# adamyindh/Multi-Step-Actor-Critic-Learning-with-Lyapunov-Certificates-for-Exponentially-Stabilizing-Control

Measured on NVIDIA B200. Metric: fused rollout env-steps/sec, higher is better.
Workload: dtype bf16x3 (split-bf16 tensor-core products, f32 accumulate; f32/f64 dynamics)

## Files before the change

include/msacl_b200.h:

```cpp
#ifndef MSACL_B200_H_
#define MSACL_B200_H_

#include <stdint.h>

#ifdef __cplusplus
extern "C" {
#endif

#define MSACL_ABI_VERSION 2

enum {
  MSACL_ENV_VANDERPOL = 0,
  MSACL_ENV_PENDULUM = 1,
  MSACL_ENV_DUCTEDFAN = 2,
  MSACL_ENV_TWOLINK = 3,
  MSACL_ENV_SINGLETRACKCAR = 4,
  MSACL_ENV_QUADTRACKING = 5,
  MSACL_NUM_ENVS = 6
};

enum {
  MSACL_OK = 0,
  MSACL_ERR_BAD_ENV = -1,
  MSACL_ERR_BAD_ARG = -2,
// ... 156 lines not shown
                             const float* dxq1, const float* dxq2, const float* log_alpha, const float* old_act,
                             const float* old_logp, const float* adv, float clip_coef, const float* act_low, const float* act_high,
                             float min_log_std, float max_log_std, float* grad_logits, double* sums, void* stream);
int msacl_alpha_update(float* log_alpha, const double* sums, int64_t rows, float target_entropy, float* adam_state,
                       float one_minus_beta1, float beta2, float one_minus_beta2, float step_size, float bc2_sqrt, float eps,
                       float clamp_max, float* entropy_out, const float* dyn, void* stream);
int msacl_adam_multi(int32_t count, float* const* params, const float* const* grads, float* const* exp_avg, float* const* exp_avg_sq,
                     const int64_t* numel, const int32_t* nsplit, int64_t max_numel, float one_minus_beta1, float beta2,
                     float one_minus_beta2, float step_size, float bc2_sqrt, float eps, const float* dyn, void* stream);
int msacl_adam_tick(int32_t* step, float* dyn, double lr, double beta1, double beta2, void* stream);

int msacl_ffma_probe(int32_t mode, int32_t iters, float* sink, double* flops, void* stream);

int msacl_selftest_tc_gemm(const float* A, const float* W, float* D, int32_t splits, void* stream);

int msacl_umma_probe(int32_t mode, int32_t iters, double* cycles_per_umma, void* stream);

enum {
  MSACL_CERT_NONFINITE = 1,
  MSACL_CERT_BOUND_LO = 2,
  MSACL_CERT_BOUND_HI = 4,
  MSACL_CERT_DECREASE = 8,
  MSACL_CERT_ESCAPED = 16,
  MSACL_CERT_NOT_EXP_STABLE = 32,
  MSACL_CERT_FAIL_MASK = 31,
  MSACL_CERT_MAX_HORIZON = 8192
};

enum {
  MSACL_CERT_SUM_STATES = 0,
// ... 119 lines not shown
```

multi-step-actor-critic-learning-with-lyapunov-certificates-for-exponentially-stabilizing-control_b200/_lib.py:

```python
import ctypes as C
import os

from . import build as _build

_LIB = None
ABI_VERSION = 2

c_f32p = C.POINTER(C.c_float)
c_f64p = C.POINTER(C.c_double)
c_i32p = C.POINTER(C.c_int32)
c_i64p = C.POINTER(C.c_int64)
c_u8p = C.POINTER(C.c_uint8)
vp = C.c_void_p


class EnvState(C.Structure):
    _fields_ = [("env_id", C.c_int32), ("max_step", C.c_int32), ("n", C.c_int64), ("stride", C.c_int64),
                ("sf", vp), ("sd", vp), ("step", vp), ("episode", vp), ("ep_return", vp), ("ep_len", vp),
                ("run", vp), ("seed", C.c_uint64), ("env_base", C.c_uint64)]


class Actor(C.Structure):
    _fields_ = [("w1", vp), ("b1", vp), ("w2t", vp), ("b2", vp), ("w3", vp), ("b3", vp),
                ("min_log_std", C.c_float), ("max_log_std", C.c_float)]
# ... 81 lines not shown
    "msacl_selftest_quad_polar": (C.c_int, [vp, vp, C.c_int64, C.c_float, vp]),
    "msacl_window_store": (C.c_int, [C.POINTER(Transitions), C.c_int32, C.c_int32, C.c_int64, C.POINTER(Ring), vp, vp,
                                     vp, vp]),
    "msacl_window_index_store": (C.c_int, [vp, C.c_int32, C.c_int64, C.c_int64, vp, C.c_int64, vp, vp, vp, vp]),
    "msacl_window_gather_indexed": (C.c_int, [C.POINTER(Transitions), C.c_int64, vp, vp, C.c_int64, C.POINTER(Ring), vp]),
    "msacl_ring_sample": (C.c_int, [C.POINTER(Ring), vp, C.c_uint64, C.c_uint64, C.c_int64, C.POINTER(Ring), vp, vp]),
    "msacl_window_sample_indexed": (C.c_int, [C.POINTER(Transitions), C.c_int64, vp, C.c_int64, vp, vp, C.c_int32, C.c_uint64, C.c_uint64,
                                              C.c_int64, C.POINTER(Ring), vp, vp]),
    "msacl_ring_gather": (C.c_int, [C.POINTER(Ring), vp, C.c_int64, C.POINTER(Ring), vp]),
    "msacl_q_backup": (C.c_int, [C.c_int64, vp, vp, vp, vp, vp, C.c_float, C.c_float, vp, vp]),
    "msacl_lyapunov_risk": (C.c_int, [C.c_int64, C.c_int32, C.c_int32, vp, vp, vp, vp, vp, vp, vp, vp, vp, C.c_float,
                                      C.c_float, C.c_float, C.c_float, vp, vp, vp, vp, vp, vp]),
    "msacl_stability_advantage": (C.c_int, [C.c_int64, C.c_int32, vp, vp, vp, vp, vp, vp, vp]),
    "msacl_advantage_normalize": (C.c_int, [C.c_int64, vp, vp, vp, vp]),
    "msacl_selftest_tc_gemm": (C.c_int, [vp, vp, vp, C.c_int32, vp]),
    "msacl_polyak_update": (C.c_int, [C.c_int32, vp, vp, vp, C.c_int64, C.c_float, C.c_float, vp]),
    "msacl_gemm_tc": (C.c_int, [C.POINTER(Gemm), vp]),
    "msacl_gemm_packed_b_bytes": (C.c_int64, [i32, i32]),
    "msacl_gemm_pack_b": (C.c_int, [C.POINTER(Gemm), vp, vp]),
    "msacl_colsum": (C.c_int, [vp, i64, i32, i64, i32, vp, vp]),
    "msacl_concat2": (C.c_int, [vp, i32, vp, i32, i64, vp, vp]),
    "msacl_reduce_splits": (C.c_int, [vp, i64, i32, vp, vp]),
    "msacl_tanh_gauss_rsample": (C.c_int, [i64, i32, vp, vp, vp, vp, f32, f32, vp, vp, vp]),
    "msacl_tanh_gauss_log_prob": (C.c_int, [i64, i32, vp, vp, vp, vp, f32, f32, vp, vp]),
    "msacl_tanh_gauss_log_prob_bwd": (C.c_int, [i64, i32, vp, vp, vp, vp, f32, f32, vp, i32, vp, vp]),
    "msacl_q_backup_dev_alpha": (C.c_int, [i64, vp, vp, vp, vp, vp, f32, vp, vp, vp]),
    "msacl_q_loss_grad": (C.c_int, [i64, vp, vp, vp, vp, vp, vp, vp]),
    "msacl_sumsq_bwd": (C.c_int, [i64, i32, vp, vp, vp, vp]),
    "msacl_policy_q_route": (C.c_int, [i64, vp, vp, vp, vp, vp, vp, vp, vp]),
    "msacl_policy_logits_grad": (C.c_int, [i64, i32, i32, i32, vp, vp, vp, vp, vp, vp, vp, vp, f32, vp, vp, f32, f32, vp, vp, vp]),
# ... 67 lines not shown
```

multi-step-actor-critic-learning-with-lyapunov-certificates-for-exponentially-stabilizing-control_b200/csrc/rollout_tc.cu:

```cuda
#include "env_phase.cuh"
#include "tcgen05.cuh"

namespace msacl {

#ifdef MSACL_TC_TIMING
#define TC_T0(var) const long long var = clock64()
#define TC_ACC(slot, t0) do { if (stats) atomicAdd(&stats[slot], (double)(clock64() - (t0))); } while (0)
#else
#define TC_T0(var) do {} while (0)
#define TC_ACC(slot, t0) do {} while (0)
#endif

#ifdef MSACL_TC_WATCHDOG
__device__ __forceinline__ void wd_wait(void* bar, uint32_t parity, int site, uint32_t aux, double* stats) {
  const long long t0 = clock64();
  uint32_t spins = 0;
  volatile unsigned long long* flag = reinterpret_cast<volatile unsigned long long*>(&stats[24]);
  while (!tc::mbar_test(bar, parity)) {
    if ((++spins & 1023u) == 0u) {
      if (*flag != 0ull) return;
      if (clock64() - t0 > 3000000000LL) {
        if (atomicCAS(reinterpret_cast<unsigned long long*>(&stats[24]), 0ull, 0x3FF0000000000000ull) == 0ull) {
          stats[25] = site; stats[26] = aux; stats[27] = blockIdx.x; stats[28] = parity; stats[29] = threadIdx.x;
          __threadfence();
// ... 15 lines not shown
constexpr int NCH = TC_HID / KC2;
constexpr int KCB = 16;
constexpr int NCHB = TC_HID / KCB;
constexpr int NB_MAX = 4;
constexpr int A_HALF = TCM * KC2 * 2;
constexpr int B_HALF = TC_HID * KCB * 2;
constexpr int A_LBO = TCM * 16, B_LBO = TC_HID * 16, SBO = 128;
constexpr int X_HALF = TCM * 16 * 2;
constexpr int W1_HALF = TC_HID * 16 * 2;
constexpr int TC_THREADS = 768, TC_ENV_REGS = 112, TC_EPI_REGS = 56, TC_MISC_REGS = 32;
constexpr int W2P_BYTES = NCHB * 2 * B_HALF;
constexpr int W1P_BYTES = 2 * W1_HALF;

struct TcBars {
  unsigned long long xfull[TC_NS], logits[TC_NS];
  unsigned long long h1full[2], h1free[2], h2full[2], h2free[2];
  unsigned long long afull[NCH], afree[NCH], bfull[NB_MAX], bfree[NB_MAX];
  uint32_t tmem_slot;
};

struct TcShare {
  int64_t first;
  int share, rounds, per, ex;
  __host__ __device__ TcShare(int64_t num_tiles, int64_t G, int64_t cta, int nt_max) {
    share = (int)(num_tiles / G + (cta < num_tiles % G ? 1 : 0));
    first = cta * (num_tiles / G) + (cta < num_tiles % G ? cta : num_tiles % G);
    rounds = (share + nt_max - 1) / nt_max;
    per = rounds ? share / rounds : 0;
    ex = rounds ? share % rounds : 0;
  }
  __host__ __device__ int tiles_in_round(int j) const { return per + (j < ex ? 1 : 0); }
// ... 3 lines not shown
template <int ID> __host__ __device__ constexpr bool tc_two_kblocks() { return Env<ID>::D + 1 > 8; }
template <int ID> __host__ __device__ constexpr int tc_ring_depth() { return tc_two_kblocks<ID>() ? 3 : 4; }
template <int ID> __host__ __device__ constexpr int tc_w3_stride() { return 2 * Env<ID>::A > 4 ? 8 : 4; }

template <int ID>
struct TcSmem {
  static constexpr bool X2 = tc_two_kblocks<ID>();
  static constexpr int NB = tc_ring_depth<ID>();
  static constexpr int XH = X2 ? X_HALF : X_HALF / 2;
  static constexpr int W1H = X2 ? W1_HALF : W1_HALF / 2;
  alignas(128) unsigned char bstage[NB][2 * B_HALF];
  alignas(128) unsigned char astage[NCH][2 * A_HALF];
  alignas(128) unsigned char w1p[2 * W1H];
  alignas(128) unsigned char xop[TC_NS][2 * XH];
  alignas(128) unsigned char zeros[X2 ? 128 : W1_HALF / 2];
  alignas(16) float w3t[TC_HID * tc_w3_stride<ID>()];
  alignas(16) float b2[TC_HID];
  alignas(16) float b3[8];
  TcBars bars;
};

typedef unsigned long long u64;
__device__ __forceinline__ u64 pack2(float lo, float hi) { u64 r; asm("mov.b64 %0, {%1, %2};" : "=l"(r) : "f"(lo), "f"(hi)); return r; }
__device__ __forceinline__ void unpack2(u64 v, float& lo, float& hi) { asm("mov.b64 {%0, %1}, %2;" : "=f"(lo), "=f"(hi) : "l"(v)); }
__device__ __forceinline__ u64 fma2(u64 a, u64 b, u64 c) { u64 d; asm("fma.rn.f32x2 %0, %1, %2, %3;" : "=l"(d) : "l"(a), "l"(b), "l"(c)); return d; }

__device__ __forceinline__ uint32_t pack_bf16x2_rn(float lo, float hi) {
  uint32_t r;
  asm("cvt.rn.bf16x2.f32 %0, %1, %2;" : "=r"(r) : "f"(hi), "f"(lo));
  return r;
}
__device__ __forceinline__ void split8(const float (&v)[8], uint4& hi, uint4& lo) {
  uint32_t h[4], l[4];
#pragma unroll
  for (int p = 0; p < 4; ++p) {
    h[p] = pack_bf16x2_rn(v[2 * p], v[2 * p + 1]);
    const float r0 = v[2 * p] - __uint_as_float(h[p] << 16);
    const float r1 = v[2 * p + 1] - __uint_as_float(h[p] & 0xFFFF0000u);
    l[p] = pack_bf16x2_rn(r0, r1);
  }
  hi = make_uint4(h[0], h[1], h[2], h[3]);
  lo = make_uint4(l[0], l[1], l[2], l[3]);
}

__global__ void tc_pack_actor_kernel(msacl_actor_t actor, int D, unsigned char* __restrict__ w1p, unsigned char* __restrict__ w2p) {
  const int gid = blockIdx.x * blockDim.x + threadIdx.x;
  if (gid < NCHB * 2 * TC_HID) {
    const int n = gid % TC_HID, kb = (gid / TC_HID) % 2, c = gid / (TC_HID * 2);
    float v[8];
#pragma unroll
    for (int j = 0; j < 8; ++j) v[j] = actor.w2t[(size_t)(c * KCB + kb * 8 + j) * TC_HID + n];
    uint4 hi, lo;
    split8(v, hi, lo);
    unsigned char* base = w2p + (size_t)c * 2 * B_HALF + kb * B_LBO + n * 16;
// ... 18 lines not shown

template <int ID>
__global__ void __launch_bounds__(TC_THREADS, 1)
rollout_tc_kernel(msacl_env_state_t st, msacl_actor_t actor, const unsigned char* __restrict__ w1p_g,
                  const unsigned char* __restrict__ w2p_g, int K, uint32_t step_base, int n_step,
                  float reward_scale, float cost_scale, const float* __restrict__ eps, int deterministic, msacl_transitions_t out,
                  double* stats) {
  using E = Env<ID>;
  using S = TcSmem<ID>;
  constexpr int D = E::D, A = E::A, A2 = 2 * A;
  constexpr int NS = TC_NS;
  constexpr int NB = S::NB, XH = S::XH, W1H = S::W1H, W3S = tc_w3_stride<ID>();
  constexpr bool X2 = S::X2;
  constexpr int W_EPI1 = 4 * NS, W_MMA = W_EPI1 + 8, W_TMA = W_MMA + 1;
  static_assert(D < 16, "layer-1 K block holds obs + bias column");
  static_assert(A2 * TCM * 4 <= XH && ((A2 + 1) / 2) * 2 * TCM * 4 <= XH, "logits and partial sums alias the two halves of the X-operand region");
  extern __shared__ __align__(128) unsigned char smem_raw[];
  S& sm = *reinterpret_cast<S*>(smem_raw);
  const int tid = threadIdx.x, lane = tid & 31, warp = tid >> 5;
  auto logits_of = [&](int s) { return reinterpret_cast<float*>(sm.xop[s]); };

  for (int i = tid; i < 2 * W1H / 16; i += TC_THREADS) {
    const int img = i / (W1H / 16), off = i % (W1H / 16);
    reinterpret_cast<uint4*>(sm.w1p)[i] = reinterpret_cast<const uint4*>(w1p_g + (size_t)img * W1_HALF)[off];
  }
  for (int i = tid; i < (int)sizeof(sm.zeros) / 16; i += TC_THREADS) reinterpret_cast<uint4*>(sm.zeros)[i] = make_uint4(0, 0, 0, 0);
  for (int i = tid; i < W3S * TC_HID; i += TC_THREADS) { const int n = i / W3S, j = i % W3S; sm.w3t[i] = j < A2 ? actor.w3[j * TC_HID + n] : 0.f; }
  for (int i = tid; i < TC_HID; i += TC_THREADS) sm.b2[i] = actor.b2[i];
  if (tid < 8) sm.b3[tid] = tid < A2 ? actor.b3[tid] : 0.f;
  if (tid == 0) {
    TcBars& b = sm.bars;
    for (int s = 0; s < NS; ++s) tc::mbar_init(&b.xfull[s], TCM);
    for (int s = 0; s < NS; ++s) tc::mbar_init(&b.logits[s], TCM);
    for (int i = 0; i < 2; ++i) {
      tc::mbar_init(&b.h1full[i], 1); tc::mbar_init(&b.h1free[i], 2 * TCM);
      tc::mbar_init(&b.h2full[i], 1); tc::mbar_init(&b.h2free[i], 2 * TCM);
    }
    for (int i = 0; i < NCH; ++i) { tc::mbar_init(&b.afull[i], TCM); tc::mbar_init(&b.afree[i], 1); }
    for (int i = 0; i < NB; ++i) { tc::mbar_init(&b.bfull[i], 1); tc::mbar_init(&b.bfree[i], 1); }
    tc::mbar_fence_init();
  }
  if (warp == W_MMA) tc::tmem_alloc(&sm.bars.tmem_slot, 512);
  tc::fence_async_smem();
  tc::tc_fence_before();
  __syncthreads();
  tc::tc_fence_after();
  const uint32_t tmem = sm.bars.tmem_slot;

  const int64_t num_tiles = (st.n + TCM - 1) / TCM;
  const int64_t G = gridDim.x, cta = blockIdx.x;
  const TcShare sh(num_tiles, G, cta, NS);
// ... 113 lines not shown
          *reinterpret_cast<uint4*>(base + kb * A_LBO) = hi;
          *reinterpret_cast<uint4*>(base + A_HALF + kb * A_LBO) = lo;
        }
        tc::fence_async_smem();
        tc::mbar_arrive(&sm.bars.afull[c]);
      }
      if (timer) TC_ACC(9, t_b);
    };
    auto epi2 = [&](uint32_t t0, int s) {
      const uint32_t buf = t0 & 1u, tmem_b = tmem + buf * 256u;
      TC_T0(t_a);
      TC_WAIT(&sm.bars.h2full[buf], (t0 >> 1) & 1, 4, t0);
      tc::tc_fence_after();
      if (timer) TC_ACC(11, t_a);
      TC_T0(t_b);
      constexpr int NP = (A2 + 1) / 2;
      u64 acc[NP];
#pragma unroll
      for (int p = 0; p < NP; ++p) acc[p] = h == 0 ? pack2(sm.b3[2 * p], sm.b3[2 * p + 1]) : pack2(0.f, 0.f);
#pragma unroll 1
      for (int cc = 0; cc < TC_HID / 32; ++cc) {
        const int cb = h * (TC_HID / 32) + cc;
        uint32_t v[16];
        tc::tmem_ld16(tmem_b + lane_addr + (uint32_t)(cb * 16), v);
        tc::tmem_ld_wait();
        if (cc == TC_HID / 32 - 1) { tc::tc_fence_before(); tc::mbar_arrive(&sm.bars.h2free[buf]); }
#pragma unroll
        for (int g = 0; g < 4; ++g) {
          const float4 bb = *reinterpret_cast<const float4*>(&sm.b2[cb * 16 + 4 * g]);
          const float hv[4] = {fmaxf(__uint_as_float(v[4 * g + 0]) + bb.x, 0.f), fmaxf(__uint_as_float(v[4 * g + 1]) + bb.y, 0.f),
                               fmaxf(__uint_as_float(v[4 * g + 2]) + bb.z, 0.f), fmaxf(__uint_as_float(v[4 * g + 3]) + bb.w, 0.f)};
#pragma unroll
          for (int c = 0; c < 4; ++c) {
            const float* wrow = &sm.w3t[(cb * 16 + 4 * g + c) * W3S];
            const u64 hh = pack2(hv[c], hv[c]);
            if constexpr (NP >= 1) {
              const float4 w0 = *reinterpret_cast<const float4*>(wrow);
              acc[0] = fma2(hh, pack2(w0.x, w0.y), acc[0]);
              if constexpr (NP >= 2) acc[1] = fma2(hh, pack2(w0.z, w0.w), acc[1]);
            }
            if constexpr (NP >= 3) {
              const float4 w1 = *reinterpret_cast<const float4*>(wrow + 4);
              acc[2] = fma2(hh, pack2(w1.x, w1.y), acc[2]);
              if constexpr (NP >= 4) acc[3] = fma2(hh, pack2(w1.z, w1.w), acc[3]);
            }
          }
        }
      }
      float* part = reinterpret_cast<float*>(sm.xop[s] + XH);
      float* lgs = logits_of(s);
      if (h == 1) {
#pragma unroll
        for (int p = 0; p < NP; ++p) {
          float lo, hi;
          unpack2(acc[p], lo, hi);
          part[(2 * p) * TCM + r] = lo;
          part[(2 * p + 1) * TCM + r] = hi;
        }
      }
      tc::bar_sync(4 + q, 64);
      if (h == 0) {
#pragma unroll
        for (int p = 0; p < NP; ++p) {
          float lo, hi;
          unpack2(acc[p], lo, hi);
          lgs[(2 * p) * TCM + r] = lo + part[(2 * p) * TCM + r];
          if (2 * p + 1 < A2) lgs[(2 * p + 1) * TCM + r] = hi + part[(2 * p + 1) * TCM + r];
        }
        tc::mbar_arrive(&sm.bars.logits[s]);
      }
      if (timer) TC_ACC(12, t_b);
    };
    uint32_t ts = 0;
    for (int64_t pair = blockIdx.x; pair < num_pairs; pair += gridDim.x) {
      const int nt = tiles_in_pair(pair);
      for (int k = 0; k < K; ++k)
        for (int s = 0; s < nt; ++s, ++ts) {
          if (ts == 0) epi1(0u);
          const bool has_next = !(s + 1 == nt && k + 1 == K && pair + (int64_t)gridDim.x >= num_pairs);
          const bool epi2_first = nt <= 1;
          if (!epi2_first) {
            if (has_next) epi1(ts + 1);
            epi2(ts, s);
          } else {
            epi2(ts, s);
            if (has_next) epi1(ts + 1);
// ... 18 lines not shown
        TC_T0(t_x);
        TC_WAIT(&sm.bars.xfull[s % NS], xn & 1, 7, t1);
        TC_ACC(13, t_x);
        tc::tc_fence_after();
        const uint32_t tmem_b = tmem + (t1 & 1u) * 256u;
        const uint32_t xbase = tc::smem_u32(sm.xop[s % NS]), zbase = tc::smem_u32(sm.zeros);
        const uint64_t dw1 = tc::make_smem_desc(w1base, X2 ? B_LBO : zbase - w1base, SBO);
        const uint64_t dw2 = tc::make_smem_desc(w1base + W1H, X2 ? B_LBO : zbase - (w1base + W1H), SBO);
        const uint64_t dx1 = tc::make_smem_desc(xbase, X2 ? A_LBO : zbase - xbase, SBO);
        const uint64_t dx2 = tc::make_smem_desc(xbase + XH, X2 ? A_LBO : zbase - (xbase + XH), SBO);
        tc::umma_bf16(tmem_b, dx1, dw1, idesc, 0u);
        tc::umma_bf16(tmem_b, dx1, dw2, idesc, 1u);
        tc::umma_bf16(tmem_b, dx2, dw1, idesc, 1u);
        tc::umma_commit(&sm.bars.h1full[t1 & 1]);
      };
      uint32_t ts = 0, pi = 0;
      for (int64_t pair = blockIdx.x; pair < num_pairs; pair += gridDim.x, ++pi) {
        const int nt = tiles_in_pair(pair);
        for (int k = 0; k < K; ++k)
          for (int s = 0; s < nt; ++s, ++ts) {
            if (ts == 0) issue_l1(0, 0u, 0u);
            const uint32_t buf = ts & 1u, tmem_b = tmem + buf * 256u;
            int s2 = s + 1, k2 = k;
            int64_t pair2 = pair;
            uint32_t pi2 = pi;
            if (s2 == nt) { s2 = 0; if (++k2 == K) { k2 = 0; pair2 += gridDim.x; ++pi2; } }
            bool next_pending = pair2 < num_pairs;
            const uint32_t xn2 = x_index(pi2, k2, s2, (pair2 == pair || !next_pending) ? nt : tiles_in_pair(pair2)), t2 = ts + 1;
            auto try_next = [&]() {
              if (next_pending && (t2 < 2 || tc::mbar_test(&sm.bars.h2free[t2 & 1], ((t2 >> 1) - 1) & 1)) &&
                  tc::mbar_test(&sm.bars.xfull[s2 % NS], xn2 & 1)) {
                issue_l1(s2, xn2, t2);
                next_pending = false;
              }
            };
            try_next();
            TC_T0(t_h);
            TC_WAIT(&sm.bars.h1free[buf], (ts >> 1) & 1, 8, ts);
            TC_ACC(14, t_h);
#pragma unroll 1
            for (int c = 0; c < NCH; ++c) {
              TC_T0(t_1);
              TC_WAIT(&sm.bars.afull[c], ts & 1, 9, ts);
              TC_ACC(15, t_1);
              const uint32_t a_lo = a_lo0 + (uint32_t)c * (2 * A_HALF / 16);
#pragma unroll
              for (int j = 0; j < KC2 / KCB; ++j) {
                TC_T0(t_2);
                TC_WAIT(&sm.bars.bfull[bs], bph, 11, ts);
                TC_ACC(16, t_2);
                tc::tc_fence_after();
                const uint32_t b_lo = b_lo0 + bs * (2 * B_HALF / 16);
                const uint64_t da1 = mk(a_lo + j * (2 * A_LBO / 16)), da2 = mk(a_lo + j * (2 * A_LBO / 16) + A_HALF / 16);
                const uint64_t db1 = mk(b_lo), db2 = mk(b_lo + B_HALF / 16);
                tc::umma_bf16(tmem_b, da1, db1, idesc, (c > 0 || j > 0) ? 1u : 0u);
                tc::umma_bf16(tmem_b, da1, db2, idesc, 1u);
                tc::umma_bf16(tmem_b, da2, db1, idesc, 1u);
                tc::umma_commit(&sm.bars.bfree[bs]);
                if (++bs == NB) { bs = 0; bph ^= 1u; }
              }
              tc::umma_commit(&sm.bars.afree[c]);
              try_next();
            }
            tc::umma_commit(&sm.bars.h2full[buf]);
            if (next_pending) issue_l1(s2, xn2, t2);
#ifdef MSACL_TC_TIMING
            if (stats) atomicAdd(&stats[18], 1.0);
#endif
          }
      }
    }
    } else if (warp == W_TMA) {
    if (tc::elect_one()) {
      int64_t tile_steps = 0;
      for (int64_t pair = blockIdx.x; pair < num_pairs; pair += gridDim.x) tile_steps += (int64_t)tiles_in_pair(pair) * K;
      const int64_t total = tile_steps * NCHB;
      uint32_t bs = 0, bph = 1, kk = 0;
      for (int64_t i = 0; i < total; ++i) {
        if (i >= NB) TC_WAIT(&sm.bars.bfree[bs], bph, 13, i);
// ... 66 lines not shown
```

multi-step-actor-critic-learning-with-lyapunov-certificates-for-exponentially-stabilizing-control_b200/csrc/tc_selftest.cu:

```cuda
#include "common.cuh"
#include "tcgen05.cuh"

namespace msacl {

constexpr int ST_M = 128, ST_N = 256, ST_K = 256, ST_KC = 64;

__global__ void __launch_bounds__(128, 1)
tc_gemm_selftest_kernel(const float* __restrict__ A, const float* __restrict__ W, float* __restrict__ D, int splits) {
  extern __shared__ __align__(128) unsigned char smem[];
  unsigned char* a1 = smem;
  unsigned char* a2 = smem + 65536;
  unsigned char* b1 = smem + 131072;
  unsigned char* b2 = smem + 131072 + 32768;
  unsigned long long* bar = reinterpret_cast<unsigned long long*>(smem + 196608);
  uint32_t* tmem_slot = reinterpret_cast<uint32_t*>(smem + 196608 + 64);
  const int tid = threadIdx.x, warp = tid >> 5, lane = tid & 31;

  if (tid == 0) { tc::mbar_init(bar, 1); tc::mbar_fence_init(); }
  if (warp == 0) tc::tmem_alloc(tmem_slot, 256);
  tc::tc_fence_before();
  __syncthreads();
  tc::tc_fence_after();
  const uint32_t tmem = *tmem_slot;

// ... 39 lines not shown
    tc::mbar_wait(bar, (uint32_t)(c & 1));
    tc::tc_fence_after();
  }
  for (int cb = 0; cb < ST_N / 32; ++cb) {
    uint32_t r[32];
    tc::tmem_ld32(tmem + ((uint32_t)(warp * 32) << 16) + (uint32_t)(cb * 32), r);
    tc::tmem_ld_wait();
#pragma unroll
    for (int j = 0; j < 32; ++j) D[(warp * 32 + lane) * ST_N + cb * 32 + j] = __uint_as_float(r[j]);
  }
  tc::tc_fence_before();
  __syncthreads();
  if (warp == 0) tc::tmem_dealloc(tmem, 256);
}

__global__ void __launch_bounds__(256, 1) umma_probe_kernel(int mode, int iters, double* __restrict__ out) {
  extern __shared__ __align__(128) unsigned char smem[];
  unsigned char* a = smem;
  unsigned char* b = smem + 131072;
  unsigned char* scratch = smem + 180224;
  unsigned long long* bar = reinterpret_cast<unsigned long long*>(smem + 204800);
  uint32_t* tmem_slot = reinterpret_cast<uint32_t*>(smem + 204800 + 64);
  volatile int* stop = reinterpret_cast<volatile int*>(smem + 204800 + 128);
  const int tid = threadIdx.x, warp = tid >> 5;
  unsigned long long* ldcount = reinterpret_cast<unsigned long long*>(smem + 204800 + 192);
  for (int i = tid; i < 180224 / 16; i += 256) reinterpret_cast<uint4*>(smem)[i] = make_uint4(0, 0, 0, 0);
  if (tid == 0) { tc::mbar_init(bar, 1); tc::mbar_init(bar + 1, 1); tc::mbar_init(bar + 2, 1); tc::mbar_fence_init(); tc::mbar_arrive(bar + 2); *stop = 0; *ldcount = 0ull; }
  if (warp == 0) tc::tmem_alloc(tmem_slot, 512);
  tc::fence_async_smem();
  tc::tc_fence_before();
  __syncthreads();
  tc::tc_fence_after();
  const uint32_t tmem = *tmem_slot;
  if (tid == 0) {
    const uint32_t idesc = tc::make_idesc_bf16(128, 256);
    const long long t0 = clock64();
    for (int i = 0; i < iters; ++i) {
      const uint32_t ab = tc::smem_u32(a + ((i >> 1) & 7) * 16384 + (i & 1) * 4096), bb = tc::smem_u32(b + (i % 3) * 16384);
      const uint64_t da1 = tc::make_smem_desc(ab, 2048, 128), da2 = tc::make_smem_desc(ab + 8192, 2048, 128);
      const uint64_t db1 = tc::make_smem_desc(bb, 4096, 128), db2 = tc::make_smem_desc(bb + 8192, 4096, 128);
      tc::umma_bf16(tmem, da1, db1, idesc, i > 0 ? 1u : 0u);
      tc::umma_bf16(tmem, da1, db2, idesc, 1u);
      tc::umma_bf16(tmem, da2, db1, idesc, 1u);
      if (mode >= 3) tc::umma_commit(bar + 1);
      if (mode >= 4) { tc::mbar_wait(bar + 2, 0u); tc::tc_fence_after(); }
    }
    tc::umma_commit(bar);
    tc::mbar_wait(bar, 0u);
    const long long t1 = clock64();
    *stop = 1;
    if (blockIdx.x == 0) { out[0] = (double)(t1 - t0) / (3.0 * iters); out[2] = (double)(t1 - t0); }
  } else if (warp > 0 && warp < 4 && mode == 1) {
    uint4 v = make_uint4(tid, tid, tid, tid);
    int off = (tid - 32) * 16;
    while (!*stop) {
#pragma unroll
      for (int q = 0; q < 8; ++q) *reinterpret_cast<uint4*>(scratch + ((off + q * 1536) % 24576)) = v;
      off = (off + 12288) % 24576;
    }
  } else if (warp > 0 && mode == 2) {
    unsigned long long n = 0;
    uint32_t acc = 0;
    while (!*stop) {
#pragma unroll 1
      for (int cb = 0; cb < 8; ++cb) {
        uint32_t v[32];
// ... 6 lines not shown
    }
    if (acc == 0x12345678u) out[3] = 1.0;
    if ((tid & 31) == 0) atomicAdd(ldcount, n);
  }
  tc::tc_fence_before();
  __syncthreads();
  if (tid == 0 && blockIdx.x == 0 && mode == 2) out[1] = (double)(*ldcount) * 4096.0 / out[2];
  if (warp == 0) tc::tmem_dealloc(tmem, 512);
}

}

using namespace msacl;

extern "C" int msacl_umma_probe(int32_t mode, int32_t iters, double* cycles_per_umma, void* stream) {
  if (!cycles_per_umma || iters <= 0 || mode < 0 || mode > 4) { set_error("umma_probe: bad argument"); return MSACL_ERR_BAD_ARG; }
  const int smem = 204800 + 256;
  cudaError_t e = cudaFuncSetAttribute(umma_probe_kernel, cudaFuncAttributeMaxDynamicSharedMemorySize, smem);
  if (e != cudaSuccess) { set_error("umma_probe: %s", cudaGetErrorString(e)); return MSACL_ERR_CUDA; }
  umma_probe_kernel<<<kNumSMs, 256, smem, (cudaStream_t)stream>>>(mode, iters, cycles_per_umma);
  return check_launch("umma_probe");
}

extern "C" int msacl_selftest_tc_gemm(const float* A, const float* W, float* D, int32_t splits, void* stream) {
  if (!A || !W || !D || (splits != 1 && splits != 3)) { set_error("selftest_tc_gemm: bad argument"); return MSACL_ERR_BAD_ARG; }
  const int smem = 196608 + 128;
  cudaError_t e = cudaFuncSetAttribute(tc_gemm_selftest_kernel, cudaFuncAttributeMaxDynamicSharedMemorySize, smem);
  if (e != cudaSuccess) { set_error("selftest_tc_gemm: %s", cudaGetErrorString(e)); return MSACL_ERR_CUDA; }
  tc_gemm_selftest_kernel<<<1, 128, smem, (cudaStream_t)stream>>>(A, W, D, splits);
  return check_launch("selftest_tc_gemm");
}
```

multi-step-actor-critic-learning-with-lyapunov-certificates-for-exponentially-stabilizing-control_b200/csrc/tcgen05.cuh:

```cuda
#pragma once
#include <cstdint>

namespace msacl {
namespace tc {

__device__ __forceinline__ uint32_t smem_u32(const void* p) { return (uint32_t)__cvta_generic_to_shared(p); }

__device__ __forceinline__ bool elect_one() {
  uint32_t pred;
  asm volatile(
      "{\n\t"
      ".reg .pred p;\n\t"
      "elect.sync _|p, 0xffffffff;\n\t"
      "selp.u32 %0, 1, 0, p;\n\t"
      "}" : "=r"(pred));
  return pred != 0;
}

__device__ __forceinline__ void mbar_init(void* bar, uint32_t count) {
  asm volatile("mbarrier.init.shared::cta.b64 [%0], %1;" ::"r"(smem_u32(bar)), "r"(count) : "memory");
}
__device__ __forceinline__ void mbar_fence_init() {
  asm volatile("fence.mbarrier_init.release.cluster;" ::: "memory");
}
// ... 57 lines not shown
}
__host__ __device__ constexpr uint32_t make_idesc_bf16(int M, int N) {
  return (1u << 4)
         | (1u << 7) | (1u << 10)
         | ((uint32_t)(N >> 3) << 17)
         | ((uint32_t)(M >> 4) << 24);
}

__device__ __forceinline__ void umma_bf16(uint32_t tmem_d, uint64_t a_desc, uint64_t b_desc, uint32_t idesc, uint32_t accumulate) {
  asm volatile(
      "{\n\t"
      ".reg .pred p;\n\t"
      "setp.ne.b32 p, %4, 0;\n\t"
      "tcgen05.mma.cta_group::1.kind::f16 [%0], %1, %2, %3, p;\n\t"
      "}" ::"r"(tmem_d), "l"(a_desc), "l"(b_desc), "r"(idesc), "r"(accumulate) : "memory");
}
__device__ __forceinline__ void umma_commit(void* bar) {
  asm volatile("tcgen05.commit.cta_group::1.mbarrier::arrive::one.shared::cluster.b64 [%0];" ::"r"(smem_u32(bar)) : "memory");
}

__device__ __forceinline__ void tmem_ld32(uint32_t taddr, uint32_t (&r)[32]) {
  asm volatile(
      "tcgen05.ld.sync.aligned.32x32b.x32.b32 "
      "{%0, %1, %2, %3, %4, %5, %6, %7, %8, %9, %10, %11, %12, %13, %14, %15, "
      "%16, %17, %18, %19, %20, %21, %22, %23, %24, %25, %26, %27, %28, %29, %30, %31}, [%32];"
      : "=r"(r[0]), "=r"(r[1]), "=r"(r[2]), "=r"(r[3]), "=r"(r[4]), "=r"(r[5]), "=r"(r[6]), "=r"(r[7]), "=r"(r[8]),
        "=r"(r[9]), "=r"(r[10]), "=r"(r[11]), "=r"(r[12]), "=r"(r[13]), "=r"(r[14]), "=r"(r[15]), "=r"(r[16]),
        "=r"(r[17]), "=r"(r[18]), "=r"(r[19]), "=r"(r[20]), "=r"(r[21]), "=r"(r[22]), "=r"(r[23]), "=r"(r[24]),
        "=r"(r[25]), "=r"(r[26]), "=r"(r[27]), "=r"(r[28]), "=r"(r[29]), "=r"(r[30]), "=r"(r[31])
      : "r"(taddr)
// ... 10 lines not shown
}
__device__ __forceinline__ void tmem_ld8(uint32_t taddr, uint32_t (&r)[8]) {
  asm volatile(
      "tcgen05.ld.sync.aligned.32x32b.x8.b32 {%0, %1, %2, %3, %4, %5, %6, %7}, [%8];"
      : "=r"(r[0]), "=r"(r[1]), "=r"(r[2]), "=r"(r[3]), "=r"(r[4]), "=r"(r[5]), "=r"(r[6]), "=r"(r[7])
      : "r"(taddr)
      : "memory");
}
__device__ __forceinline__ void tmem_ld_wait() { asm volatile("tcgen05.wait::ld.sync.aligned;" ::: "memory"); }
__device__ __forceinline__ void tmem_st8(uint32_t taddr, const uint32_t (&r)[8]) {
  asm volatile(
      "tcgen05.st.sync.aligned.32x32b.x8.b32 [%0], {%1, %2, %3, %4, %5, %6, %7, %8};"
      ::"r"(taddr), "r"(r[0]), "r"(r[1]), "r"(r[2]), "r"(r[3]), "r"(r[4]), "r"(r[5]), "r"(r[6]), "r"(r[7])
      : "memory");
}
__device__ __forceinline__ void tmem_st_wait() { asm volatile("tcgen05.wait::st.sync.aligned;" ::: "memory"); }

__device__ __forceinline__ uint32_t f32_to_bf16_bits(float x) {
  uint32_t u = __float_as_uint(x);
  u += 0x7FFFu + ((u >> 16) & 1u);
  return u >> 16;
}
__device__ __forceinline__ void split_bf16(float x, uint32_t& hi, uint32_t& lo) {
  hi = f32_to_bf16_bits(x);
  const float r = x - __uint_as_float(hi << 16);
  lo = f32_to_bf16_bits(r);
}

}
}
```

Baseline: 2.155 billion.

## Move actor layer-3 matmul onto tensor cores with TMEM A-operand

Replaces the CUDA-core FMA loop for the actor's third layer with tcgen05 MMAs. The epilogue warps apply bias and ReLU to layer-2 outputs, split them into bf16 hi/lo, and store them back into TMEM. The MMA warp then issues M=128,N=16 MMAs with TMEM as the A operand against a packed hi/lo W3 image in shared memory. The first K block is still done on CUDA cores in the slot where the accumulator lands. New l3full/l3done barriers and opportunistic issue points in the MMA loop add synchronisation and extra tensor-core work. This trades epilogue FMA cost for TMEM round trips and serialization risk.

```diff
diff --git a/include/msacl_b200.h b/include/msacl_b200.h
--- a/include/msacl_b200.h
+++ b/include/msacl_b200.h
@@ -194,6 +194,8 @@
 
 int msacl_selftest_tc_gemm(const float* A, const float* W, float* D, int32_t splits, void* stream);
 
+int msacl_selftest_tc_layer3(const float* H, const float* W, int32_t n_out, float* out, void* stream);
+
 int msacl_umma_probe(int32_t mode, int32_t iters, double* cycles_per_umma, void* stream);
 
 enum {
diff --git a/multi-step-actor-critic-learning-with-lyapunov-certificates-for-exponentially-stabilizing-control_b200/_lib.py b/multi-step-actor-critic-learning-with-lyapunov-certificates-for-exponentially-stabilizing-control_b200/_lib.py
--- a/multi-step-actor-critic-learning-with-lyapunov-certificates-for-exponentially-stabilizing-control_b200/_lib.py
+++ b/multi-step-actor-critic-learning-with-lyapunov-certificates-for-exponentially-stabilizing-control_b200/_lib.py
@@ -119,6 +119,7 @@
     "msacl_stability_advantage": (C.c_int, [C.c_int64, C.c_int32, vp, vp, vp, vp, vp, vp, vp]),
     "msacl_advantage_normalize": (C.c_int, [C.c_int64, vp, vp, vp, vp]),
     "msacl_selftest_tc_gemm": (C.c_int, [vp, vp, vp, C.c_int32, vp]),
+    "msacl_selftest_tc_layer3": (C.c_int, [vp, vp, C.c_int32, vp, vp]),
     "msacl_polyak_update": (C.c_int, [C.c_int32, vp, vp, vp, C.c_int64, C.c_float, C.c_float, vp]),
     "msacl_gemm_tc": (C.c_int, [C.POINTER(Gemm), vp]),
     "msacl_gemm_packed_b_bytes": (C.c_int64, [i32, i32]),
diff --git a/multi-step-actor-critic-learning-with-lyapunov-certificates-for-exponentially-stabilizing-control_b200/csrc/rollout_tc.cu b/multi-step-actor-critic-learning-with-lyapunov-certificates-for-exponentially-stabilizing-control_b200/csrc/rollout_tc.cu
--- a/multi-step-actor-critic-learning-with-lyapunov-certificates-for-exponentially-stabilizing-control_b200/csrc/rollout_tc.cu
+++ b/multi-step-actor-critic-learning-with-lyapunov-certificates-for-exponentially-stabilizing-control_b200/csrc/rollout_tc.cu
@@ -53,7 +53,7 @@
 
 struct TcBars {
   unsigned long long xfull[TC_NS], logits[TC_NS];
-  unsigned long long h1full[2], h1free[2], h2full[2], h2free[2];
+  unsigned long long h1full[2], h1free[2], h2full[2], h2free[2], l3full[2], l3done[2];
   unsigned long long afull[NCH], afree[NCH], bfull[NB_MAX], bfree[NB_MAX];
   uint32_t tmem_slot;
 };
@@ -87,7 +87,8 @@
   alignas(128) unsigned char w1p[2 * W1H];
   alignas(128) unsigned char xop[TC_NS][2 * XH];
   alignas(128) unsigned char zeros[X2 ? 128 : W1_HALF / 2];
-  alignas(16) float w3t[TC_HID * tc_w3_stride<ID>()];
+  alignas(128) unsigned char w3b[(tc::L3_BLOCKS - 1) * tc::L3_B_BYTES];
+  alignas(16) float w3k0[tc::L3_KB * tc_w3_stride<ID>()];
   alignas(16) float b2[TC_HID];
   alignas(16) float b3[8];
   TcBars bars;
@@ -98,19 +99,14 @@
 __device__ __forceinline__ void unpack2(u64 v, float& lo, float& hi) { asm("mov.b64 {%0, %1}, %2;" : "=f"(lo), "=f"(hi) : "l"(v)); }
 __device__ __forceinline__ u64 fma2(u64 a, u64 b, u64 c) { u64 d; asm("fma.rn.f32x2 %0, %1, %2, %3;" : "=l"(d) : "l"(a), "l"(b), "l"(c)); return d; }
 
-__device__ __forceinline__ uint32_t pack_bf16x2_rn(float lo, float hi) {
-  uint32_t r;
-  asm("cvt.rn.bf16x2.f32 %0, %1, %2;" : "=r"(r) : "f"(hi), "f"(lo));
-  return r;
-}
 __device__ __forceinline__ void split8(const float (&v)[8], uint4& hi, uint4& lo) {
   uint32_t h[4], l[4];
 #pragma unroll
   for (int p = 0; p < 4; ++p) {
-    h[p] = pack_bf16x2_rn(v[2 * p], v[2 * p + 1]);
+    h[p] = tc::pack_bf16x2_rn(v[2 * p], v[2 * p + 1]);
     const float r0 = v[2 * p] - __uint_as_float(h[p] << 16);
     const float r1 = v[2 * p + 1] - __uint_as_float(h[p] & 0xFFFF0000u);
-    l[p] = pack_bf16x2_rn(r0, r1);
+    l[p] = tc::pack_bf16x2_rn(r0, r1);
   }
   hi = make_uint4(h[0], h[1], h[2], h[3]);
   lo = make_uint4(l[0], l[1], l[2], l[3]);
@@ -159,7 +155,7 @@
   constexpr bool X2 = S::X2;
   constexpr int W_EPI1 = 4 * NS, W_MMA = W_EPI1 + 8, W_TMA = W_MMA + 1;
   static_assert(D < 16, "layer-1 K block holds obs + bias column");
-  static_assert(A2 * TCM * 4 <= XH && ((A2 + 1) / 2) * 2 * TCM * 4 <= XH, "logits and partial sums alias the two halves of the X-operand region");
+  static_assert(A2 <= 8 && A2 * TCM * 4 <= 2 * XH, "layer-3 outputs fit the accumulator's rows 0-7 and the logits the X-operand region");
   extern __shared__ __align__(128) unsigned char smem_raw[];
   S& sm = *reinterpret_cast<S*>(smem_raw);
   const int tid = threadIdx.x, lane = tid & 31, warp = tid >> 5;
@@ -170,7 +166,8 @@
     reinterpret_cast<uint4*>(sm.w1p)[i] = reinterpret_cast<const uint4*>(w1p_g + (size_t)img * W1_HALF)[off];
   }
   for (int i = tid; i < (int)sizeof(sm.zeros) / 16; i += TC_THREADS) reinterpret_cast<uint4*>(sm.zeros)[i] = make_uint4(0, 0, 0, 0);
-  for (int i = tid; i < W3S * TC_HID; i += TC_THREADS) { const int n = i / W3S, j = i % W3S; sm.w3t[i] = j < A2 ? actor.w3[j * TC_HID + n] : 0.f; }
+  for (int i = tid; i < W3S * tc::L3_KB; i += TC_THREADS) { const int n = i / W3S, j = i % W3S; sm.w3k0[i] = j < A2 ? actor.w3[j * TC_HID + n] : 0.f; }
+  tc::l3_fill_b(sm.w3b, actor.w3, A2, tid, TC_THREADS);
   for (int i = tid; i < TC_HID; i += TC_THREADS) sm.b2[i] = actor.b2[i];
   if (tid < 8) sm.b3[tid] = tid < A2 ? actor.b3[tid] : 0.f;
   if (tid == 0) {
@@ -179,7 +176,8 @@
     for (int s = 0; s < NS; ++s) tc::mbar_init(&b.logits[s], TCM);
     for (int i = 0; i < 2; ++i) {
       tc::mbar_init(&b.h1full[i], 1); tc::mbar_init(&b.h1free[i], 2 * TCM);
-      tc::mbar_init(&b.h2full[i], 1); tc::mbar_init(&b.h2free[i], 2 * TCM);
+      tc::mbar_init(&b.h2full[i], 1); tc::mbar_init(&b.h2free[i], TCM);
+      tc::mbar_init(&b.l3full[i], 2 * TCM); tc::mbar_init(&b.l3done[i], 1);
     }
     for (int i = 0; i < NCH; ++i) { tc::mbar_init(&b.afull[i], TCM); tc::mbar_init(&b.afree[i], 1); }
     for (int i = 0; i < NB; ++i) { tc::mbar_init(&b.bfull[i], 1); tc::mbar_init(&b.bfree[i], 1); }
@@ -323,25 +321,40 @@
       tc::tc_fence_after();
       if (timer) TC_ACC(11, t_a);
       TC_T0(t_b);
-      constexpr int NP = (A2 + 1) / 2;
-      u64 acc[NP];
-#pragma unroll
-      for (int p = 0; p < NP; ++p) acc[p] = h == 0 ? pack2(sm.b3[2 * p], sm.b3[2 * p + 1]) : pack2(0.f, 0.f);
 #pragma unroll 1
-      for (int cc = 0; cc < TC_HID / 32; ++cc) {
-        const int cb = h * (TC_HID / 32) + cc;
+      for (int cb = h == 0 ? 1 : tc::L3_BLOCKS / 2; cb < (h + 1) * (tc::L3_BLOCKS / 2); ++cb) {
         uint32_t v[16];
         tc::tmem_ld16(tmem_b + lane_addr + (uint32_t)(cb * 16), v);
         tc::tmem_ld_wait();
-        if (cc == TC_HID / 32 - 1) { tc::tc_fence_before(); tc::mbar_arrive(&sm.bars.h2free[buf]); }
+        float hv[16];
 #pragma unroll
         for (int g = 0; g < 4; ++g) {
           const float4 bb = *reinterpret_cast<const float4*>(&sm.b2[cb * 16 + 4 * g]);
+          hv[4 * g + 0] = fmaxf(__uint_as_float(v[4 * g + 0]) + bb.x, 0.f);
+          hv[4 * g + 1] = fmaxf(__uint_as_float(v[4 * g + 1]) + bb.y, 0.f);
+          hv[4 * g + 2] = fmaxf(__uint_as_float(v[4 * g + 2]) + bb.z, 0.f);
+          hv[4 * g + 3] = fmaxf(__uint_as_float(v[4 * g + 3]) + bb.w, 0.f);
+        }
+        tc::l3_split16(hv, v);
+        tc::tmem_st16(tmem_b + lane_addr + (uint32_t)(cb * 16), v);
+      }
+      float* lgs = logits_of(s);
+      if (h == 0) {
+        constexpr int NP = (A2 + 1) / 2;
+        u64 acc[NP];
+        uint32_t v[16];
+        tc::tmem_ld16(tmem_b + lane_addr, v);
+        tc::tmem_ld_wait();
+#pragma unroll
+        for (int p = 0; p < NP; ++p) acc[p] = pack2(sm.b3[2 * p], sm.b3[2 * p + 1]);
+#pragma unroll
+        for (int g = 0; g < 4; ++g) {
+          const float4 bb = *reinterpret_cast<const float4*>(&sm.b2[4 * g]);
           const float hv[4] = {fmaxf(__uint_as_float(v[4 * g + 0]) + bb.x, 0.f), fmaxf(__uint_as_float(v[4 * g + 1]) + bb.y, 0.f),
                                fmaxf(__uint_as_float(v[4 * g + 2]) + bb.z, 0.f), fmaxf(__uint_as_float(v[4 * g + 3]) + bb.w, 0.f)};
 #pragma unroll
           for (int c = 0; c < 4; ++c) {
-            const float* wrow = &sm.w3t[(cb * 16 + 4 * g + c) * W3S];
+            const float* wrow = &sm.w3k0[(4 * g + c) * W3S];
             const u64 hh = pack2(hv[c], hv[c]);
             if constexpr (NP >= 1) {
               const float4 w0 = *reinterpret_cast<const float4*>(wrow);
@@ -355,30 +368,32 @@
             }
           }
         }
-      }
-      float* part = reinterpret_cast<float*>(sm.xop[s] + XH);
-      float* lgs = logits_of(s);
-      if (h == 1) {
 #pragma unroll
         for (int p = 0; p < NP; ++p) {
           float lo, hi;
           unpack2(acc[p], lo, hi);
-          part[(2 * p) * TCM + r] = lo;
-          part[(2 * p + 1) * TCM + r] = hi;
-        }
-      }
-      tc::bar_sync(4 + q, 64);
+          lgs[(2 * p) * TCM + r] = lo;
+          if (2 * p + 1 < A2) lgs[(2 * p + 1) * TCM + r] = hi;
+        }
+      }
+      tc::tmem_st_wait();
+      tc::tc_fence_before();
+      tc::mbar_arrive(&sm.bars.l3full[buf]);
+      if (timer) TC_ACC(12, t_b);
       if (h == 0) {
-#pragma unroll
-        for (int p = 0; p < NP; ++p) {
-          float lo, hi;
-          unpack2(acc[p], lo, hi);
-          lgs[(2 * p) * TCM + r] = lo + part[(2 * p) * TCM + r];
-          if (2 * p + 1 < A2) lgs[(2 * p + 1) * TCM + r] = hi + part[(2 * p + 1) * TCM + r];
-        }
+        TC_T0(t_c);
+        TC_WAIT(&sm.bars.l3done[buf], (t0 >> 1) & 1, 5, t0);
+        tc::tc_fence_after();
+        if (timer) TC_ACC(19, t_c);
+        uint32_t d[16];
+        tc::tmem_ld16(tmem_b + lane_addr, d);
+        tc::tmem_ld_wait();
+        tc::tc_fence_before();
+        tc::mbar_arrive(&sm.bars.h2free[buf]);
+#pragma unroll
+        for (int j = 0; j < A2; ++j) lgs[j * TCM + r] += __uint_as_float(d[j]) + __uint_as_float(d[8 + j]);
         tc::mbar_arrive(&sm.bars.logits[s]);
       }
-      if (timer) TC_ACC(12, t_b);
     };
     uint32_t ts = 0;
     for (int64_t pair = blockIdx.x; pair < num_pairs; pair += gridDim.x) {
@@ -427,6 +442,28 @@
         tc::umma_bf16(tmem_b, dx2, dw1, idesc, 1u);
         tc::umma_commit(&sm.bars.h1full[t1 & 1]);
       };
+      const uint32_t w3b = tc::smem_u32(sm.w3b);
+      uint32_t l3n = 0;
+      auto issue_l3 = [&]() {
+        tc::tc_fence_after();
+        tc::l3_issue(tmem + (l3n & 1u) * 256u, w3b);
+        tc::umma_commit(&sm.bars.l3done[l3n & 1u]);
+        ++l3n;
+      };
+      auto try_l3 = [&](uint32_t end) {
+        if (l3n < end && tc::mbar_test(&sm.bars.l3full[l3n & 1u], (l3n >> 1) & 1)) issue_l3();
+      };
+      auto force_l3 = [&](uint32_t end) {
+        while (l3n < end) {
+          TC_T0(t_3);
+          TC_WAIT(&sm.bars.l3full[l3n & 1u], (l3n >> 1) & 1, 6, l3n);
+          TC_ACC(20, t_3);
+#ifdef MSACL_TC_TIMING
+          if (stats) atomicAdd(&stats[21], 1.0);
+#endif
+          issue_l3();
+        }
+      };
       uint32_t ts = 0, pi = 0;
       for (int64_t pair = blockIdx.x; pair < num_pairs; pair += gridDim.x, ++pi) {
         const int nt = tiles_in_pair(pair);
@@ -448,6 +485,7 @@
               }
             };
             try_next();
+            try_l3(ts);
             TC_T0(t_h);
             TC_WAIT(&sm.bars.h1free[buf], (ts >> 1) & 1, 8, ts);
             TC_ACC(14, t_h);
@@ -474,8 +512,10 @@
               }
               tc::umma_commit(&sm.bars.afree[c]);
               try_next();
+              try_l3(ts);
             }
             tc::umma_commit(&sm.bars.h2full[buf]);
+            force_l3(nt >= 2 && pair2 < num_pairs ? ts : ts + 1);
             if (next_pending) issue_l1(s2, xn2, t2);
 #ifdef MSACL_TC_TIMING
             if (stats) atomicAdd(&stats[18], 1.0);
diff --git a/multi-step-actor-critic-learning-with-lyapunov-certificates-for-exponentially-stabilizing-control_b200/csrc/tc_selftest.cu b/multi-step-actor-critic-learning-with-lyapunov-certificates-for-exponentially-stabilizing-control_b200/csrc/tc_selftest.cu
--- a/multi-step-actor-critic-learning-with-lyapunov-certificates-for-exponentially-stabilizing-control_b200/csrc/tc_selftest.cu
+++ b/multi-step-actor-critic-learning-with-lyapunov-certificates-for-exponentially-stabilizing-control_b200/csrc/tc_selftest.cu
@@ -77,6 +77,54 @@
   if (warp == 0) tc::tmem_dealloc(tmem, 256);
 }
 
+__global__ void __launch_bounds__(128, 1)
+tc_layer3_selftest_kernel(const float* __restrict__ H, const float* __restrict__ W, int N, float* __restrict__ out) {
+  __shared__ __align__(128) unsigned char bimg[(tc::L3_BLOCKS - 1) * tc::L3_B_BYTES];
+  __shared__ __align__(8) unsigned long long bar;
+  __shared__ uint32_t tmem_slot;
+  const int tid = threadIdx.x, warp = tid >> 5;
+  tc::l3_fill_b(bimg, W, N, tid, 128);
+  if (tid == 0) { tc::mbar_init(&bar, 1); tc::mbar_fence_init(); }
+  if (warp == 0) tc::tmem_alloc(&tmem_slot, 256);
+  tc::fence_async_smem();
+  tc::tc_fence_before();
+  __syncthreads();
+  tc::tc_fence_after();
+  const uint32_t tmem = tmem_slot, lane_addr = (uint32_t)(warp * 32) << 16;
+  const float* h = H + tid * tc::L3_K;
+  float part[8];
+#pragma unroll
+  for (int j = 0; j < 8; ++j) {
+    part[j] = 0.f;
+    for (int k = 0; k < tc::L3_KB; ++k) part[j] = j < N ? __fmaf_rn(h[k], W[j * tc::L3_K + k], part[j]) : 0.f;
+  }
+  for (int c = 1; c < tc::L3_BLOCKS; ++c) {
+    float v[16];
+    uint32_t img[16];
+#pragma unroll
+    for (int k = 0; k < 16; ++k) v[k] = h[c * tc::L3_KB + k];
+    tc::l3_split16(v, img);
+    tc::tmem_st16(tmem + lane_addr + (uint32_t)(c * 16), img);
+  }
+  tc::tmem_st_wait();
+  tc::tc_fence_before();
+  __syncthreads();
+  if (tid == 0) {
+    tc::tc_fence_after();
+    tc::l3_issue(tmem, tc::smem_u32(bimg));
+    tc::umma_commit(&bar);
+  }
+  tc::mbar_wait(&bar, 0u);
+  tc::tc_fence_after();
+  uint32_t d[16];
+  tc::tmem_ld16(tmem + lane_addr, d);
+  tc::tmem_ld_wait();
+  for (int j = 0; j < N; ++j) out[tid * N + j] = part[j] + (__uint_as_float(d[j]) + __uint_as_float(d[8 + j]));
+  tc::tc_fence_before();
+  __syncthreads();
+  if (warp == 0) tc::tmem_dealloc(tmem, 256);
+}
+
 __global__ void __launch_bounds__(256, 1) umma_probe_kernel(int mode, int iters, double* __restrict__ out) {
   extern __shared__ __align__(128) unsigned char smem[];
   unsigned char* a = smem;
@@ -98,7 +146,13 @@
   if (tid == 0) {
     const uint32_t idesc = tc::make_idesc_bf16(128, 256);
     const long long t0 = clock64();
-    for (int i = 0; i < iters; ++i) {
+    for (int i = 0; i < iters && mode == 5; ++i) {
+      const uint64_t db = tc::make_smem_desc(tc::smem_u32(b + (i % 15) * tc::L3_B_BYTES), tc::L3_B_LBO, tc::L3_B_SBO);
+      const uint32_t col = 16u + 16u * (uint32_t)(i % 15);
+      tc::umma_bf16_tmem_a(tmem, tmem + col, db, tc::make_idesc_bf16(128, 16), i > 0 ? 1u : 0u);
+      tc::umma_bf16_tmem_a(tmem, tmem + col + 8u, db, tc::make_idesc_bf16(128, 16), 1u);
+    }
+    for (int i = 0; i < iters && mode != 5; ++i) {
       const uint32_t ab = tc::smem_u32(a + ((i >> 1) & 7) * 16384 + (i & 1) * 4096), bb = tc::smem_u32(b + (i % 3) * 16384);
       const uint64_t da1 = tc::make_smem_desc(ab, 2048, 128), da2 = tc::make_smem_desc(ab + 8192, 2048, 128);
       const uint64_t db1 = tc::make_smem_desc(bb, 4096, 128), db2 = tc::make_smem_desc(bb + 8192, 4096, 128);
@@ -112,7 +166,7 @@
     tc::mbar_wait(bar, 0u);
     const long long t1 = clock64();
     *stop = 1;
-    if (blockIdx.x == 0) { out[0] = (double)(t1 - t0) / (3.0 * iters); out[2] = (double)(t1 - t0); }
+    if (blockIdx.x == 0) { out[0] = (double)(t1 - t0) / ((mode == 5 ? 2.0 : 3.0) * iters); out[2] = (double)(t1 - t0); }
   } else if (warp > 0 && warp < 4 && mode == 1) {
     uint4 v = make_uint4(tid, tid, tid, tid);
     int off = (tid - 32) * 16;
@@ -149,7 +203,7 @@
 using namespace msacl;
 
 extern "C" int msacl_umma_probe(int32_t mode, int32_t iters, double* cycles_per_umma, void* stream) {
-  if (!cycles_per_umma || iters <= 0 || mode < 0 || mode > 4) { set_error("umma_probe: bad argument"); return MSACL_ERR_BAD_ARG; }
+  if (!cycles_per_umma || iters <= 0 || mode < 0 || mode > 5) { set_error("umma_probe: bad argument"); return MSACL_ERR_BAD_ARG; }
   const int smem = 204800 + 256;
   cudaError_t e = cudaFuncSetAttribute(umma_probe_kernel, cudaFuncAttributeMaxDynamicSharedMemorySize, smem);
   if (e != cudaSuccess) { set_error("umma_probe: %s", cudaGetErrorString(e)); return MSACL_ERR_CUDA; }
@@ -165,3 +219,9 @@
   tc_gemm_selftest_kernel<<<1, 128, smem, (cudaStream_t)stream>>>(A, W, D, splits);
   return check_launch("selftest_tc_gemm");
 }
+
+extern "C" int msacl_selftest_tc_layer3(const float* H, const float* W, int32_t n_out, float* out, void* stream) {
+  if (!H || !W || !out || n_out < 1 || n_out > 8) { set_error("selftest_tc_layer3: bad argument"); return MSACL_ERR_BAD_ARG; }
+  tc_layer3_selftest_kernel<<<1, 128, 0, (cudaStream_t)stream>>>(H, W, n_out, out);
+  return check_launch("selftest_tc_layer3");
+}
diff --git a/multi-step-actor-critic-learning-with-lyapunov-certificates-for-exponentially-stabilizing-control_b200/csrc/tcgen05.cuh b/multi-step-actor-critic-learning-with-lyapunov-certificates-for-exponentially-stabilizing-control_b200/csrc/tcgen05.cuh
--- a/multi-step-actor-critic-learning-with-lyapunov-certificates-for-exponentially-stabilizing-control_b200/csrc/tcgen05.cuh
+++ b/multi-step-actor-critic-learning-with-lyapunov-certificates-for-exponentially-stabilizing-control_b200/csrc/tcgen05.cuh
@@ -95,6 +95,14 @@
       "setp.ne.b32 p, %4, 0;\n\t"
       "tcgen05.mma.cta_group::1.kind::f16 [%0], %1, %2, %3, p;\n\t"
       "}" ::"r"(tmem_d), "l"(a_desc), "l"(b_desc), "r"(idesc), "r"(accumulate) : "memory");
+}
+__device__ __forceinline__ void umma_bf16_tmem_a(uint32_t tmem_d, uint32_t tmem_a, uint64_t b_desc, uint32_t idesc, uint32_t accumulate) {
+  asm volatile(
+      "{\n\t"
+      ".reg .pred p;\n\t"
+      "setp.ne.b32 p, %4, 0;\n\t"
+      "tcgen05.mma.cta_group::1.kind::f16 [%0], [%1], %2, %3, p;\n\t"
+      "}" ::"r"(tmem_d), "r"(tmem_a), "l"(b_desc), "r"(idesc), "r"(accumulate) : "memory");
 }
 __device__ __forceinline__ void umma_commit(void* bar) {
   asm volatile("tcgen05.commit.cta_group::1.mbarrier::arrive::one.shared::cluster.b64 [%0];" ::"r"(smem_u32(bar)) : "memory");
@@ -135,8 +143,21 @@
       ::"r"(taddr), "r"(r[0]), "r"(r[1]), "r"(r[2]), "r"(r[3]), "r"(r[4]), "r"(r[5]), "r"(r[6]), "r"(r[7])
       : "memory");
 }
+__device__ __forceinline__ void tmem_st16(uint32_t taddr, const uint32_t (&r)[16]) {
+  asm volatile(
+      "tcgen05.st.sync.aligned.32x32b.x16.b32 [%0], "
+      "{%1, %2, %3, %4, %5, %6, %7, %8, %9, %10, %11, %12, %13, %14, %15, %16};"
+      ::"r"(taddr), "r"(r[0]), "r"(r[1]), "r"(r[2]), "r"(r[3]), "r"(r[4]), "r"(r[5]), "r"(r[6]), "r"(r[7]), "r"(r[8]),
+        "r"(r[9]), "r"(r[10]), "r"(r[11]), "r"(r[12]), "r"(r[13]), "r"(r[14]), "r"(r[15])
+      : "memory");
+}
 __device__ __forceinline__ void tmem_st_wait() { asm volatile("tcgen05.wait::st.sync.aligned;" ::: "memory"); }
 
+__device__ __forceinline__ uint32_t pack_bf16x2_rn(float lo, float hi) {
+  uint32_t r;
+  asm("cvt.rn.bf16x2.f32 %0, %1, %2;" : "=r"(r) : "f"(hi), "f"(lo));
+  return r;
+}
 __device__ __forceinline__ uint32_t f32_to_bf16_bits(float x) {
   uint32_t u = __float_as_uint(x);
   u += 0x7FFFu + ((u >> 16) & 1u);
@@ -148,5 +169,42 @@
   lo = f32_to_bf16_bits(r);
 }
 
-}
-}
+constexpr int L3_K = 256, L3_KB = 16, L3_BLOCKS = L3_K / L3_KB;
+constexpr int L3_B_BYTES = 512, L3_B_LBO = 256, L3_B_SBO = 128;
+
+__device__ __forceinline__ void l3_split16(const float (&v)[16], uint32_t (&img)[16]) {
+#pragma unroll
+  for (int p = 0; p < 8; ++p) {
+    const uint32_t hi = pack_bf16x2_rn(v[2 * p], v[2 * p + 1]);
+    img[p] = hi;
+    img[8 + p] = pack_bf16x2_rn(v[2 * p] - __uint_as_float(hi << 16), v[2 * p + 1] - __uint_as_float(hi & 0xFFFF0000u));
+  }
+}
+
+__device__ inline void l3_fill_b(unsigned char* dst, const float* __restrict__ W, int N, int i0, int di) {
+  for (int i = i0; i < (L3_BLOCKS - 1) * 32; i += di) {
+    const int c = 1 + i / 32, n = (i >> 1) & 15, kh = i & 1, j = n & 7;
+    uint32_t w[4];
+#pragma unroll
+    for (int p = 0; p < 4; ++p) {
+      const int k = c * L3_KB + kh * 8 + 2 * p;
+      const float a = j < N ? W[j * L3_K + k] : 0.f, b = j < N ? W[j * L3_K + k + 1] : 0.f;
+      const uint32_t hi = pack_bf16x2_rn(a, b);
+      w[p] = n < 8 ? hi : pack_bf16x2_rn(a - __uint_as_float(hi << 16), b - __uint_as_float(hi & 0xFFFF0000u));
+    }
+    *reinterpret_cast<uint4*>(dst + (c - 1) * L3_B_BYTES + kh * L3_B_LBO + n * 16) = make_uint4(w[0], w[1], w[2], w[3]);
+  }
+}
+
+__device__ __forceinline__ void l3_issue(uint32_t tmem_acc, uint32_t b_smem) {
+  constexpr uint32_t idesc = make_idesc_bf16(128, 16);
+  uint64_t db = make_smem_desc(b_smem, L3_B_LBO, L3_B_SBO);
+#pragma unroll 1
+  for (uint32_t c = 1; c < L3_BLOCKS; ++c, db += L3_B_BYTES / 16) {
+    umma_bf16_tmem_a(tmem_acc, tmem_acc + 16u * c, db, idesc, c > 1 ? 1u : 0u);
+    umma_bf16_tmem_a(tmem_acc, tmem_acc + 16u * c + 8u, db, idesc, 1u);
+  }
+}
+
+}
+}
```

Result: slower. 2.125 billion (median of 6 runs) (-1.4%).
